# jabhinav/Semi-Supervised-Gated-LT-VAE

Measured on NVIDIA B200. Metric: training images/sec (sup+unsup ELBO step), higher is better.
Workload: dtype bf16

## Files before the change

semi-supervised-gated-lt-vae_b200/csrc/conv_tc.cu:

```cuda
#include <stdlib.h>
#include <string.h>

#include <mutex>
#include <type_traits>

#include "common.cuh"
#include "tc_common.cuh"

namespace gccvae {
using namespace tc;

__device__ __forceinline__ size_t s2d_slot(int n, int y, int x, int H, int W) {
  const int HB = (H >> 1) + 1, WB = (W >> 1) + 1;
  return (((size_t)n * HB + ((y + 1) >> 1)) * WB + ((x + 1) >> 1)) * 4 + (((y + 1) & 1) * 2 + ((x + 1) & 1));
}

struct alignas(64) TapGemmParams {
  CUtensorMap tmA, tmB;
  int num_taps, chunks, KC, swz;
  int a_scale;
  int BW, BH, BN;
  int tiles_w, tiles_h;
  int N, n_store;
  int b_tap_stride;
  short a_dw[4][16], a_dh[4][16];
  int b_row0[4];
  void* out;
  const void* mask;
  const float* bias;
  int bias_mod;
  int act;
  int out_f32;
  int OH, OW, OC, oys, oxs;
  int oy0[4], ox0[4];
  int batch;
  int stages;
  int tps;
  int n_slabs;
  int phases;
  int total_items;
  int bias_n;
  long long* timeline;
  int out_s2d, mask_s2d;
  int rows_valid;
  int pad_;
  int halo2;
  int a_box_rows;
};

#ifdef GCCVAE_TIMELINE
#define TL_ON(p) ((p).timeline != nullptr)
#define TL(item_local, slot)                                                              \
  do {                                                                                    \
    if (p.timeline != nullptr && blockIdx.x == 0 && (item_local) < 32)                    \
      p.timeline[(item_local) * 8 + (slot)] = clock64();                                  \
  } while (0)
#else
#define TL_ON(p) false
#define TL(item_local, slot) \
  do {                       \
  } while (0)
#endif

constexpr int TG_THREADS = 192;

__global__ void __launch_bounds__(TG_THREADS) tapgemm_kernel(const __grid_constant__ TapGemmParams p) {
  extern __shared__ uint8_t smem_raw[];
  const uint32_t base = (smem_u32(smem_raw) + 1023u) & ~1023u;
  uint8_t* smem = smem_raw + (base - smem_u32(smem_raw));
  const int a_bytes = p.a_box_rows * p.KC * 2, b_tile = p.N * p.KC * 2, b_bytes = (p.halo2 ? 2 : 1) * b_tile;
  const int a_stride = (a_bytes + 1023) & ~1023, b_stride = (b_bytes + 1023) & ~1023;
  const int stage_stride = p.tps * (a_stride + b_stride);
  uint8_t* sA = smem;
  uint8_t* sB = smem + p.tps * a_stride;
  uint64_t* full = reinterpret_cast<uint64_t*>(smem + p.stages * stage_stride);
  uint64_t* empty = full + p.stages;
  uint64_t* tfull = empty + p.stages;
  uint64_t* tempty = tfull + 2;
  uint32_t* tmem_slot = reinterpret_cast<uint32_t*>(tempty + 2);
  float* s_bias = reinterpret_cast<float*>((reinterpret_cast<uintptr_t>(tmem_slot + 4) + 15) & ~(uintptr_t)15);

  const int warp = threadIdx.x >> 5, lane = threadIdx.x & 31;
  pdl_launch_dependents();
  const int per_cta = (p.total_items + (int)gridDim.x - 1) / (int)gridDim.x;
  const int item_beg = blockIdx.x * per_cta;
  const int item_end = min(item_beg + per_cta, p.total_items);
  const int tiles_per_group = p.tiles_w * p.tiles_h;
  uint32_t acc_cols = 32;
  while ((int)acc_cols < p.N) acc_cols <<= 1;
  const uint32_t tmem_cols = acc_cols * 2;

  if (warp == 0 && lane == 0) {
    tma_prefetch_desc(&p.tmA);
    tma_prefetch_desc(&p.tmB);
    for (int s = 0; s < p.stages; ++s) {
      mbar_init(&full[s], 1);
      mbar_init(&empty[s], 1);
    }
    for (int s = 0; s < 2; ++s) {
      mbar_init(&tfull[s], 1);
      mbar_init(&tempty[s], 4);
    }
    fence_mbar_init();
  }
  if (warp == 2) tmem_alloc(tmem_slot, tmem_cols);
  tc_fence_before();
  __syncthreads();
  tc_fence_after();
  const uint32_t tmem_base = *tmem_slot;
  pdl_wait();
  if (TL_ON(p) && threadIdx.x == 0 && blockIdx.x < 1024) {
    unsigned long long gt;
    asm volatile("mov.u64 %0, %globaltimer;" : "=l"(gt));
    p.timeline[40 * 8 + 2 * blockIdx.x] = (long long)gt;
  }

  const int k_iters = p.num_taps * p.chunks;
  if (warp == 0) {
    if (elect_one()) {
      int stage = 0;
      uint32_t ph = 0;
      long long prod_wait = 0;
      const long long tp0 = clock64();
      const uint32_t stage_tx =
          (uint32_t)(p.tps * ((p.halo2 ? p.a_box_rows : p.rows_valid) * p.KC * 2 + b_bytes));
      for (int item = item_beg; item < item_end; ++item) {
        const int phase_id = item % p.phases, slab = (item / p.phases) % p.n_slabs, tile = item / (p.phases * p.n_slabs);
        const int grp = tile / tiles_per_group, tin = tile % tiles_per_group;
        const int w0 = (tin % p.tiles_w) * p.BW, h0 = (tin / p.tiles_w) * p.BH, n0 = grp * p.BN;
        const int aw = p.a_scale * w0, ah = p.a_scale * h0, brow = p.b_row0[phase_id] + slab * p.N;
        int t = 0, c = 0;
        for (int it = 0; it < k_iters; it += p.tps) {
          const long long tw0 = TL_ON(p) ? clock64() : 0;
          mbar_wait(&empty[stage], ph ^ 1);
          if (TL_ON(p)) prod_wait += clock64() - tw0;
          if (it == 0) TL(item - item_beg, 0);
          mbar_expect_tx(&full[stage], stage_tx);
          uint8_t* a_dst = sA + stage * stage_stride;
          uint8_t* b_dst = sB + stage * stage_stride;
          for (int j = 0; j < p.tps; ++j) {
            tma_load_4d(a_dst, &p.tmA, &full[stage], c * p.KC, aw + p.a_dw[phase_id][t], ah + p.a_dh[phase_id][t], n0);
            if (p.halo2) {
              tma_load_2d(b_dst, &p.tmB, &full[stage], t * p.b_tap_stride + c * p.KC, brow);
              tma_load_2d(b_dst + b_tile, &p.tmB, &full[stage], (2 + t) * p.b_tap_stride + c * p.KC, brow);
            } else {
              tma_load_2d(b_dst, &p.tmB, &full[stage], t * p.b_tap_stride + c * p.KC, brow);
            }
            a_dst += a_stride;
            b_dst += b_stride;
            if (++c == p.chunks) { c = 0; ++t; }
          }
          if (it + p.tps >= k_iters) TL(item - item_beg, 1);
          if (++stage == p.stages) { stage = 0; ph ^= 1; }
        }
      }
      if (TL_ON(p) && blockIdx.x == 0) {
        p.timeline[32 * 8 + 0] = prod_wait;
        p.timeline[32 * 8 + 1] = clock64() - tp0;
      }
    }
  } else if (warp == 1) {
    if (lane == 0) {
      const uint32_t idesc = instr_desc_bf16(128, p.N, 0, 0);
      const uint32_t sbo = 8u * (uint32_t)p.KC * 2u;
      const uint64_t dproto = smem_desc(0, 16, sbo, (uint32_t)p.swz);
      const uint64_t adesc0 = dproto + (uint64_t)(smem_u32(sA) >> 4), bdesc0 = dproto + (uint64_t)(smem_u32(sB) >> 4);
      const uint32_t a_step = (uint32_t)a_stride >> 4, b_step = (uint32_t)b_stride >> 4;
      const uint32_t st_step = (uint32_t)stage_stride >> 4;
      const int kk_n = p.KC / 16;
      int stage = 0;
      uint32_t ph = 0;
      long long mma_wait = 0, acc_wait = 0;
      const long long tm0 = clock64();
      auto run = [&](auto kk_c) {
      constexpr int KK = decltype(kk_c)::value;
      for (int item = item_beg; item < item_end; ++item) {
        const int li = item - item_beg, as = li & 1;
        const long long ta0 = TL_ON(p) ? clock64() : 0;
        mbar_wait(&tempty[as], ((uint32_t)(li >> 1) & 1u) ^ 1u);
        if (TL_ON(p)) acc_wait += clock64() - ta0;
        tc_fence_after();
        TL(li, 2);
        const uint32_t tacc = tmem_base + (uint32_t)as * acc_cols;
        for (int it = 0; it < k_iters; it += p.tps) {
          const long long tw0 = TL_ON(p) ? clock64() : 0;
          mbar_wait(&full[stage], ph);
          if (TL_ON(p)) mma_wait += clock64() - tw0;
          tc_fence_after();
          if (it + p.tps >= k_iters) TL(li, 3);
          uint64_t ad = adesc0 + (uint64_t)((uint32_t)stage * st_step);
          uint64_t bd = bdesc0 + (uint64_t)((uint32_t)stage * st_step);
          if (p.halo2) {
            const uint32_t a_shift = (uint32_t)(p.BW * p.KC * 2) >> 4, b_shift = (uint32_t)b_tile >> 4;
            for (int j = 0; j < p.tps; ++j) {
              for (int a = 0; a < 2; ++a)
#pragma unroll
                for (int kk = 0; kk < KK; ++kk)
                  umma_bf16(tacc, ad + (uint64_t)(a * a_shift + 2u * kk), bd + (uint64_t)(a * b_shift + 2u * kk), idesc,
                            (it > 0 || j > 0 || a > 0 || kk > 0) ? 1u : 0u);
              ad += a_step;
              bd += b_step;
            }
          } else {
          umma_bf16(tacc, ad, bd, idesc, it > 0 ? 1u : 0u);
#pragma unroll
          for (int kk = 1; kk < KK; ++kk) umma_bf16(tacc, ad + 2u * kk, bd + 2u * kk, idesc, 1u);
          for (int j = 1; j < p.tps; ++j) {
            ad += a_step;
            bd += b_step;
#pragma unroll
            for (int kk = 0; kk < KK; ++kk) umma_bf16(tacc, ad + 2u * kk, bd + 2u * kk, idesc, 1u);
          }
          }
          umma_commit(&empty[stage]);
          if (it + p.tps >= k_iters) umma_commit(&tfull[as]);
          if (++stage == p.stages) { stage = 0; ph ^= 1; }
        }
      }
      };
      if (kk_n == 4) run(std::integral_constant<int, 4>{});
      else if (kk_n == 2) run(std::integral_constant<int, 2>{});
      else run(std::integral_constant<int, 1>{});
      if (TL_ON(p) && blockIdx.x == 0) {
        p.timeline[32 * 8 + 2] = mma_wait;
        p.timeline[32 * 8 + 3] = acc_wait;
        p.timeline[32 * 8 + 4] = clock64() - tm0;
        p.timeline[32 * 8 + 5] = (long long)(item_end - item_beg) * (k_iters / p.tps);
        p.timeline[32 * 8 + 6] = p.stages;
        p.timeline[32 * 8 + 7] = gridDim.x;
      }
    }
  } else {
    const int q = warp & 3;
    const int m = q * 32 + lane;
    const int dx = m % p.BW, dy = (m / p.BW) % p.BH, dn = m / (p.BW * p.BH);
    {
      const int nb = p.bias == nullptr ? 0 : (p.bias_mod < p.bias_n ? p.bias_mod : p.bias_n);
      for (int i = threadIdx.x - 64; i < 256; i += 128) s_bias[i] = i < nb ? p.bias[i] : 0.0f;
      asm volatile("bar.sync 1, 128;" ::: "memory");
    }
    for (int item = item_beg; item < item_end; ++item) {
      const int li = item - item_beg, as = li & 1;
      const int phase_id = item % p.phases, slab = (item / p.phases) % p.n_slabs, tile = item / (p.phases * p.n_slabs);
      const int grp = tile / tiles_per_group, tin = tile % tiles_per_group;
      const int w0 = (tin % p.tiles_w) * p.BW, h0 = (tin / p.tiles_w) * p.BH, n0 = grp * p.BN;
      const int slab0 = slab * p.N;
      const int n = n0 + dn, y = h0 + dy, x = w0 + dx;
      const bool valid = n < p.batch && m < p.rows_valid;
      const int oyy = y * p.oys + p.oy0[phase_id], oxx = x * p.oxs + p.ox0[phase_id];
      const size_t opix_lin = ((size_t)n * p.OH + (size_t)oyy) * p.OW + oxx;
      const size_t opix_s2d = (p.out_s2d | p.mask_s2d) ? s2d_slot(n, oyy, oxx, p.OH, p.OW) : 0;
      const size_t opix = p.out_s2d ? opix_s2d : opix_lin;
      const size_t mpix = p.mask_s2d ? opix_s2d : opix_lin;
      const uint32_t tacc = tmem_base + (uint32_t)as * acc_cols + ((uint32_t)(q * 32) << 16);
      uint32_t mpre[4][8];
      const bool use_mask = p.mask != nullptr && valid;
      if (use_mask) {
        const __nv_bfloat16* mk = reinterpret_cast<const __nv_bfloat16*>(p.mask) + mpix * p.OC + slab0;
#pragma unroll
        for (int i = 0; i < 4; ++i)
          if (i * 16 < p.N && slab0 + i * 16 < p.n_store) ld_global_nc_256(mk + i * 16, mpre[i]);
      }
      mbar_wait(&tfull[as], (uint32_t)(li >> 1) & 1u);
      tc_fence_after();
      if (threadIdx.x == 64) TL(li, 4);
      const int bias_base = slab0 % p.bias_mod;
      const uint32_t s_bias_u32 = smem_u32(s_bias);
      for (int c0 = 0; c0 < p.N; c0 += 16) {
        const int cg = slab0 + c0;
        const uint32_t bsrc = s_bias_u32 + (uint32_t)(((bias_base + c0) & 255) * 4);
        uint32_t r[16];
        tmem_ld16(tacc + (uint32_t)c0, r);
        tmem_ld_wait();
        if (c0 + 16 >= p.N) {
          tc_fence_before();
          if (lane == 0) mbar_arrive(&tempty[as]);
          if (threadIdx.x == 64) TL(li, 5);
        }
        if (!valid || cg >= p.n_store) continue;
        float v[16];
#pragma unroll
        for (int i = 0; i < 4; ++i) {
          const float4 t = lds_f4(bsrc + 16u * i);
          v[4 * i] = __uint_as_float(r[4 * i]) + t.x;
          v[4 * i + 1] = __uint_as_float(r[4 * i + 1]) + t.y;
          v[4 * i + 2] = __uint_as_float(r[4 * i + 2]) + t.z;
          v[4 * i + 3] = __uint_as_float(r[4 * i + 3]) + t.w;
        }
        if (p.act == GCCVAE_ACT_RELU) {
#pragma unroll
          for (int i = 0; i < 16; ++i) v[i] = fmaxf(v[i], 0.0f);
        } else if (p.act == GCCVAE_ACT_SIGMOID) {
          if (p.out_f32 == 2) {
#pragma unroll
            for (int i = 0; i < 3; ++i) v[i] = __fdividef(1.0f, 1.0f + __expf(-v[i]));
          } else {
#pragma unroll
            for (int i = 0; i < 16; ++i) v[i] = __fdividef(1.0f, 1.0f + __expf(-v[i]));
          }
        }
        const size_t o = opix * p.OC + cg;
        if (use_mask) {
          uint32_t mw[8];
          if (c0 < 64) {
            switch (c0 >> 4) {
              case 0:
#pragma unroll
                for (int i = 0; i < 8; ++i) mw[i] = mpre[0][i];
                break;
              case 1:
#pragma unroll
                for (int i = 0; i < 8; ++i) mw[i] = mpre[1][i];
                break;
              case 2:
#pragma unroll
                for (int i = 0; i < 8; ++i) mw[i] = mpre[2][i];
                break;
              default:
#pragma unroll
                for (int i = 0; i < 8; ++i) mw[i] = mpre[3][i];
                break;
            }
          } else {
            ld_global_nc_256(reinterpret_cast<const __nv_bfloat16*>(p.mask) + mpix * p.OC + cg, mw);
          }
#pragma unroll
          for (int i = 0; i < 8; ++i) {
            const uint32_t lo = mw[i] & 0xffffu, hi = mw[i] >> 16;
            if (!(lo != 0 && lo < 0x8000u)) v[2 * i] = 0.0f;
            if (!(hi != 0 && hi < 0x8000u)) v[2 * i + 1] = 0.0f;
          }
        }
        if (p.out_f32 == 2) {
          if (c0 == 0) reinterpret_cast<float4*>(p.out)[opix] = make_float4(v[0], v[1], v[2], 0.0f);
        } else if (p.out_f32) {
          float* dst = reinterpret_cast<float*>(p.out) + o;
          uint32_t w0[8], w1[8];
#pragma unroll
          for (int i = 0; i < 8; ++i) { w0[i] = __float_as_uint(v[i]); w1[i] = __float_as_uint(v[8 + i]); }
          st_global_256(dst, w0);
          st_global_256(dst + 8, w1);
        } else {
          uint32_t w[8];
#pragma unroll
          for (int i = 0; i < 8; ++i) w[i] = pack_bf16x2(v[2 * i], v[2 * i + 1]);
          st_global_256(reinterpret_cast<__nv_bfloat16*>(p.out) + o, w);
        }
      }
      if (threadIdx.x == 64) TL(li, 6);
    }
    tc_fence_before();
  }
  __syncthreads();
  if (TL_ON(p) && threadIdx.x == 0 && blockIdx.x < 1024) {
    unsigned long long gt;
    asm volatile("mov.u64 %0, %globaltimer;" : "=l"(gt));
    p.timeline[40 * 8 + 2 * blockIdx.x + 1] = (long long)gt;
  }
  if (warp == 2) {
    tc_fence_after();
    tmem_dealloc(tmem_base, tmem_cols);
  }
}

struct alignas(64) SlHaloParams {
  CUtensorMap tmA, tmB;
  int C, BW, BH, tiles_h;
  int N, n_store, swz;
  void* out;
  const void* mask;
  const float* bias;
  int bias_n, act, out_f32;
  int OH, OW, OC, batch, total_tiles, stages;
  long long* timeline;
  int mask_s2d;
};
constexpr int HALO_THREADS = 320;

__global__ void __launch_bounds__(HALO_THREADS) sl_halo_kernel(const __grid_constant__ SlHaloParams p) {
  extern __shared__ uint8_t smem_raw[];
  const uint32_t base = (smem_u32(smem_raw) + 1023u) & ~1023u;
  uint8_t* smem = smem_raw + (base - smem_u32(smem_raw));
  const int rowb = p.C * 2;
  const int avb = (p.BH + 2) * p.BW * rowb;
  const int a_stage = 3 * avb;
  const int bblk = 4 * p.N * rowb;
  uint8_t* sB = smem;
  uint8_t* sA = smem + ((9 * bblk + 1023) & ~1023);
  uint64_t* full = reinterpret_cast<uint64_t*>(sA + p.stages * a_stage);
  uint64_t* empty = full + p.stages;
  uint64_t* tfull = empty + p.stages;
  uint64_t* tempty = tfull + 2;
  uint64_t* bfull = tempty + 2;
  uint32_t* tmem_slot = reinterpret_cast<uint32_t*>(bfull + 1);
  float* s_bias = reinterpret_cast<float*>((reinterpret_cast<uintptr_t>(tmem_slot + 4) + 15) & ~(uintptr_t)15);

  const int warp = threadIdx.x >> 5, lane = threadIdx.x & 31;
  pdl_launch_dependents();
  const int per_cta = (p.total_tiles + (int)gridDim.x - 1) / (int)gridDim.x;
  const int tile_beg = blockIdx.x * per_cta;
  const int tile_end = min(tile_beg + per_cta, p.total_tiles);
  uint32_t tmem_cols = 32;
  while ((int)tmem_cols < 8 * p.N) tmem_cols <<= 1;

  if (warp == 0 && lane == 0) {
    tma_prefetch_desc(&p.tmA);
    tma_prefetch_desc(&p.tmB);
    for (int s = 0; s < p.stages; ++s) {
      mbar_init(&full[s], 1);
      mbar_init(&empty[s], 1);
    }
    for (int s = 0; s < 2; ++s) {
      mbar_init(&tfull[s], 1);
      mbar_init(&tempty[s], 8);
    }
    mbar_init(bfull, 1);
    fence_mbar_init();
  }
  if (warp == 2) tmem_alloc(tmem_slot, tmem_cols);
  for (int i = threadIdx.x; i < 256; i += HALO_THREADS)
    s_bias[i] = (p.bias != nullptr && i < p.bias_n) ? p.bias[i] : 0.0f;
  tc_fence_before();
  __syncthreads();
  tc_fence_after();
  const uint32_t tmem_base = *tmem_slot;
  pdl_wait();

  if (warp == 0) {
    if (elect_one() && tile_beg < tile_end) {
      mbar_expect_tx(bfull, (uint32_t)(9 * bblk));
      for (int view = 0; view < 9; ++view)
        tma_load_2d(sB + view * bblk, &p.tmB, bfull, 0, view * 4 * p.N);
      int stage = 0;
      uint32_t ph = 0;
      for (int tile = tile_beg; tile < tile_end; ++tile) {
        const int n = tile / p.tiles_h, h0 = (tile % p.tiles_h) * p.BH;
        mbar_wait(&empty[stage], ph ^ 1);
        TL(tile - tile_beg, 0);
        mbar_expect_tx(&full[stage], (uint32_t)a_stage);
        for (int v = 0; v < 3; ++v)
          tma_load_4d(sA + stage * a_stage + v * avb, &p.tmA, &full[stage], 0, v - 1, h0 - 1, n);
// ... 1211 lines not shown
  });
  return fn;
}

static CUtensorMapSwizzle tma_swizzle_for(int inner_bytes) {
  return inner_bytes >= 128 ? CU_TENSOR_MAP_SWIZZLE_128B
         : inner_bytes >= 64 ? CU_TENSOR_MAP_SWIZZLE_64B
         : inner_bytes >= 32 ? CU_TENSOR_MAP_SWIZZLE_32B
                             : CU_TENSOR_MAP_SWIZZLE_NONE;
}
static int umma_swizzle_for(int inner_bytes) {
  return inner_bytes >= 128 ? SW_128 : inner_bytes >= 64 ? SW_64 : inner_bytes >= 32 ? SW_32 : SW_NONE;
}

static int encode_act_map(CUtensorMap* m, const void* ptr, int N, int H, int W, int C, int kc, int bw, int bh, int bn,
                          int es) {
  EncodeTiledFn enc = get_encode();
  if (!enc) {
    set_error("cuTensorMapEncodeTiled is unavailable (driver too old?)");
    return GCCVAE_ECUDA;
  }
  cuuint64_t dims[4] = {(cuuint64_t)C, (cuuint64_t)W, (cuuint64_t)H, (cuuint64_t)N};
  cuuint64_t strides[3] = {(cuuint64_t)C * 2, (cuuint64_t)W * C * 2, (cuuint64_t)H * W * C * 2};
  cuuint32_t box[4] = {(cuuint32_t)kc, (cuuint32_t)(bw * es), (cuuint32_t)(bh * es), (cuuint32_t)bn};
  cuuint32_t estr[4] = {1, (cuuint32_t)es, (cuuint32_t)es, 1};
  CUresult r = enc(m, CU_TENSOR_MAP_DATA_TYPE_BFLOAT16, 4, const_cast<void*>(ptr), dims, strides, box, estr,
                   CU_TENSOR_MAP_INTERLEAVE_NONE, tma_swizzle_for(kc * 2), CU_TENSOR_MAP_L2_PROMOTION_L2_128B,
                   CU_TENSOR_MAP_FLOAT_OOB_FILL_NONE);
  if (r != CUDA_SUCCESS) {
    set_error("cuTensorMapEncodeTiled(act %dx%dx%dx%d box %d,%d,%d,%d es %d) failed: %d", N, H, W, C, kc, bw * es,
              bh * es, bn, es, (int)r);
    return GCCVAE_ECUDA;
  }
  return GCCVAE_OK;
}

static int encode_mat_map(CUtensorMap* m, const void* ptr, long long rows, long long K, int kc, int nrows) {
  EncodeTiledFn enc = get_encode();
  if (!enc) {
    set_error("cuTensorMapEncodeTiled is unavailable (driver too old?)");
    return GCCVAE_ECUDA;
  }
  cuuint64_t dims[2] = {(cuuint64_t)K, (cuuint64_t)rows};
  cuuint64_t strides[1] = {(cuuint64_t)K * 2};
  cuuint32_t box[2] = {(cuuint32_t)kc, (cuuint32_t)nrows};
  cuuint32_t estr[2] = {1, 1};
  CUresult r = enc(m, CU_TENSOR_MAP_DATA_TYPE_BFLOAT16, 2, const_cast<void*>(ptr), dims, strides, box, estr,
                   CU_TENSOR_MAP_INTERLEAVE_NONE, tma_swizzle_for(kc * 2), CU_TENSOR_MAP_L2_PROMOTION_L2_128B,
                   CU_TENSOR_MAP_FLOAT_OOB_FILL_NONE);
  if (r != CUDA_SUCCESS) {
    set_error("cuTensorMapEncodeTiled(mat %lldx%lld box %d,%d) failed: %d", rows, K, kc, nrows, (int)r);
    return GCCVAE_ECUDA;
  }
  return GCCVAE_OK;
}

static int pick_kc(int C) {
  if (C % 64 == 0) return 64;
  if (C == 32) return 32;
  if (C == 16) return 16;
  return 0;
}

static int pick_tile(int H, int W, int* bw, int* bh, int* bn) {
  if (W >= 128 || 128 % W != 0) return -1;
  *bw = W;
  int rest = 128 / W;
  if (H >= rest) {
    if (H % rest != 0) return -1;
    *bh = rest;
    *bn = 1;
  } else {
    if (rest % H != 0) return -1;
    *bh = H;
    *bn = rest / H;
  }
  return 0;
}

constexpr int WG_PER_SM = 2, WG_SMEM_KB = 100;

template <class Params>
static cudaError_t launch_pdl(void (*kernel)(const Params), dim3 grid, int threads, size_t smem, cudaStream_t st,
                              const Params& p) {
  cudaLaunchConfig_t cfg;
  memset(&cfg, 0, sizeof(cfg));
  cfg.gridDim = grid;
  cfg.blockDim = dim3(threads, 1, 1);
  cfg.dynamicSmemBytes = smem;
  cfg.stream = st;
  cudaLaunchAttribute attr[1];
  attr[0].id = cudaLaunchAttributeProgrammaticStreamSerialization;
  attr[0].val.programmaticStreamSerializationAllowed = 1;
  cfg.attrs = attr;
  cfg.numAttrs = 1;
  return cudaLaunchKernelEx(&cfg, kernel, p);
}

static long long* g_timeline = nullptr;

static int launch_tapgemm(TapGemmParams& p, int groups, int phases, cudaStream_t st, const char* name) {
  p.timeline = g_timeline;
  if (p.rows_valid <= 0) p.rows_valid = 128;
  if (p.a_box_rows <= 0) p.a_box_rows = 128;
  const int a_stride = (p.a_box_rows * p.KC * 2 + 1023) & ~1023,
            b_stride = ((p.halo2 ? 2 : 1) * p.N * p.KC * 2 + 1023) & ~1023;
  uint32_t acc_cols = 32;
  while ((int)acc_cols < p.N) acc_cols <<= 1;
  const int k_iters = p.num_taps * p.chunks;
  int per_sm = 2;
  if (per_sm > 512 / (2 * (int)acc_cols)) per_sm = 512 / (2 * (int)acc_cols);
  if (per_sm < 1) per_sm = 1;
  const int budget = 200 * 1024 / per_sm - 4608;
  const int stage_target = 48 * 1024;
  int tps = 1;
  for (int d = 1; d <= k_iters; ++d)
    if (k_iters % d == 0 && d * (a_stride + b_stride) <= stage_target && 2 * d * (a_stride + b_stride) <= budget) tps = d;
  p.tps = tps;
  int stages = budget / (tps * (a_stride + b_stride));
  if (stages > 8) stages = 8;
  if (stages < 2) stages = 2;
  p.stages = stages;
  const size_t smem = (size_t)stages * tps * (a_stride + b_stride) + 1024 + 256 + 2048 + 64;
  static bool attr_set = false;
  if (!attr_set) {
    GCC_CUDA(cudaFuncSetAttribute(tapgemm_kernel, cudaFuncAttributeMaxDynamicSharedMemorySize, (int)(200 * 1024)));
    attr_set = true;
  }
  GCC_REQUIRE(smem <= 200 * 1024, "%s: %zu bytes of shared memory", name, smem);
  if (p.n_slabs < 1) p.n_slabs = 1;
  if (p.bias_mod < 1 || p.bias == nullptr) p.bias_mod = 1 << 30;
  if (p.bias_n < 1) p.bias_n = p.n_store;
  GCC_REQUIRE(p.bias_mod >= p.n_store || p.bias_mod % p.N == 0, "%s: bias_mod %d incompatible with N slab %d", name,
              p.bias_mod, p.N);
  GCC_REQUIRE(p.bias == nullptr || ((uintptr_t)p.bias % 16) == 0, "%s: bias must be 16-byte aligned", name);
  p.phases = phases;
  p.total_items = groups * p.tiles_w * p.tiles_h * p.n_slabs * phases;
  static int regs_per_cta = 0;
  if (regs_per_cta == 0) {
    cudaFuncAttributes fa;
    GCC_CUDA(cudaFuncGetAttributes(&fa, tapgemm_kernel));
    const int per_warp = ((fa.numRegs + 7) / 8) * 8 * 32;
    regs_per_cta = per_warp * (TG_THREADS / 32);
  }
  int occ = 65536 / regs_per_cta;
  const int occ_smem = (int)((227 * 1024) / (smem + 1024));
  if (occ > occ_smem) occ = occ_smem;
  if (occ < 1) occ = 1;
  if (per_sm > occ) per_sm = occ;
  if (getenv("GCCVAE_DEBUG_LAUNCH"))
    fprintf(stderr, "%s: N=%d KC=%d k_iters=%d tps=%d stages=%d smem=%zu per_sm=%d (occ %d) items=%d\n", name, p.N, p.KC,
            k_iters, tps, stages, smem, per_sm, occ, p.total_items);
  int ctas = p.total_items < 148 * per_sm ? p.total_items : 148 * per_sm;
  {
    const int per_cta = (p.total_items + ctas - 1) / ctas;
    ctas = (p.total_items + per_cta - 1) / per_cta;
  }
  dim3 grid(ctas, 1, 1);
  GCC_CUDA(launch_pdl(tapgemm_kernel, grid, TG_THREADS, smem, st, p));
  GCC_CHECK_LAUNCH(name);
  return GCCVAE_OK;
}

}

using namespace gccvae;

extern "C" int gccvae_ls_bf16(const gccvae_geom* g, const void* L, const void* Wp_ls, const float* bias, int act,
                              const void* mask, void* S, int out_f32, void* stream) {
  GCC_REQUIRE(g && L && Wp_ls && S, "ls_bf16: null pointer");
  const int kc = pick_kc(g->CL);
  GCC_REQUIRE(kc > 0, "ls_bf16: CL=%d unsupported (need 16, 32 or a multiple of 64)", g->CL);
  GCC_REQUIRE(g->CS % 16 == 0 && g->CS <= 256, "ls_bf16: CS=%d must be a multiple of 16, <= 256", g->CS);
  TapGemmParams p;
  memset(&p, 0, sizeof(p));
  const bool dense = (g->HS == 1 && g->WS == 1 && g->pad == 0 && g->stride == 1);
  int rc, n_slab = g->CS;
  if (dense) {
    const int Kt = g->KH * g->KW * g->CL;
    if ((rc = encode_act_map(&p.tmA, L, g->batch, 1, 1, Kt, kc, 1, 1, 128, 1))) return rc;
    p.num_taps = 1; p.chunks = Kt / kc; p.a_scale = 1; p.BW = 1; p.BH = 1; p.BN = 128; p.tiles_w = p.tiles_h = 1;
    p.b_tap_stride = 0;
    const int m_tiles = (g->batch + 127) / 128;
    n_slab = (m_tiles < 74 && g->CS % 64 == 0 && g->CS > 64) ? 64 : g->CS;
    if ((rc = encode_mat_map(&p.tmB, Wp_ls, g->CS, Kt, kc, n_slab))) return rc;
  } else {
    GCC_REQUIRE(g->KH == 4 && g->KW == 4 && g->stride == 2 && g->pad == 1, "ls_bf16: only k4/s2/p1 or dense");
    int bw, bh, bn;
    GCC_REQUIRE(pick_tile(g->HS, g->WS, &bw, &bh, &bn) == 0, "ls_bf16: cannot tile %dx%d", g->HS, g->WS);
    if ((rc = encode_act_map(&p.tmA, L, g->batch, g->HL, g->WL, g->CL, kc, bw, bh, bn, 2))) return rc;
    p.num_taps = 16; p.chunks = g->CL / kc; p.a_scale = 2; p.BW = bw; p.BH = bh; p.BN = bn;
    p.tiles_w = g->WS / bw; p.tiles_h = g->HS / bh;
    for (int t = 0; t < 16; ++t) { p.a_dh[0][t] = (short)(t / 4 - 1); p.a_dw[0][t] = (short)(t % 4 - 1); }
    p.b_tap_stride = g->CL;
    if ((rc = encode_mat_map(&p.tmB, Wp_ls, g->CS, 16LL * g->CL, kc, g->CS))) return rc;
  }
  p.KC = kc; p.swz = umma_swizzle_for(kc * 2);
  p.N = n_slab; p.n_store = g->CS; p.n_slabs = g->CS / n_slab;
  p.out = S; p.mask = mask; p.bias = bias; p.act = act & ~GCCVAE_LAYOUT_FLAGS; p.out_f32 = out_f32;
  p.out_s2d = (act & GCCVAE_OUT_S2D) ? 1 : 0; p.mask_s2d = (act & GCCVAE_MASK_S2D) ? 1 : 0;
  GCC_REQUIRE(!p.out_s2d || (out_f32 == 0 && !dense), "ls_bf16: s2d output needs a bf16 spatial output");
  p.OH = g->HS; p.OW = g->WS; p.OC = g->CS; p.oys = p.oxs = 1;
  p.batch = g->batch;
  const int groups = (g->batch + p.BN - 1) / p.BN;
  return launch_tapgemm(p, groups, 1, (cudaStream_t)stream, "ls_bf16");
}

extern "C" int gccvae_sl_bf16(const gccvae_geom* g, const void* S, const void* Wp_sl, const float* bias, int act,
                              const void* mask, void* L, int out_f32, void* stream) {
  GCC_REQUIRE(g && S && Wp_sl && L, "sl_bf16: null pointer");
  const int kc = pick_kc(g->CS);
  GCC_REQUIRE(kc > 0, "sl_bf16: CS=%d unsupported (need 16, 32 or a multiple of 64)", g->CS);
  TapGemmParams p;
  memset(&p, 0, sizeof(p));
  int rc, phases;
  const bool dense = (g->HS == 1 && g->WS == 1 && g->pad == 0 && g->stride == 1);
  if (dense) {
    const int Nt = g->KH * g->KW * g->CL;
    const int nslab = Nt <= 256 ? Nt : (Nt % 256 == 0 ? 256 : (Nt % 128 == 0 ? 128 : 0));
    GCC_REQUIRE(nslab > 0 && nslab % 16 == 0, "sl_bf16(dense): N=%d unsupported", Nt);
    phases = 1;
    if ((rc = encode_act_map(&p.tmA, S, g->batch, 1, 1, g->CS, kc, 1, 1, 128, 1))) return rc;
    p.num_taps = 1; p.chunks = g->CS / kc; p.a_scale = 1; p.BW = 1; p.BH = 1; p.BN = 128; p.tiles_w = p.tiles_h = 1;
    if ((rc = encode_mat_map(&p.tmB, Wp_sl, Nt, g->CS, kc, nslab))) return rc;
    p.N = nslab; p.n_store = Nt; p.n_slabs = Nt / nslab;
    p.OH = 1; p.OW = 1; p.OC = Nt; p.oys = p.oxs = 1;
    p.bias_mod = g->CL;
  } else {
    GCC_REQUIRE(g->KH == 4 && g->KW == 4 && g->stride == 2 && g->pad == 1, "sl_bf16: only k4/s2/p1 or dense");
    int bw, bh, bn;
    GCC_REQUIRE(pick_tile(g->HS, g->WS, &bw, &bh, &bn) == 0, "sl_bf16: cannot tile %dx%d", g->HS, g->WS);
    const int rows_pad = (g->CL + 15) / 16 * 16;
    GCC_REQUIRE(rows_pad <= 256, "sl_bf16: CL too large");
    GCC_REQUIRE(g->CL % 16 == 0 || (g->CL == 3 && out_f32 == 2 && mask == nullptr),
                "sl_bf16: CL=%d must be a multiple of 16 (or 3 with the float4 image output)", g->CL);
    phases = 4;
    if ((rc = encode_act_map(&p.tmA, S, g->batch, g->HS, g->WS, g->CS, kc, bw, bh, bn, 1))) return rc;
    p.num_taps = 4; p.chunks = g->CS / kc; p.a_scale = 1; p.BW = bw; p.BH = bh; p.BN = bn;
    p.tiles_w = g->WS / bw; p.tiles_h = g->HS / bh;
    for (int z = 0; z < 4; ++z) {
      const int ph = z >> 1, pw = z & 1;
      for (int t = 0; t < 4; ++t) { p.a_dh[z][t] = (short)(ph - (t >> 1)); p.a_dw[z][t] = (short)(pw - (t & 1)); }
// ... 579 lines not shown
```

semi-supervised-gated-lt-vae_b200/csrc/tc_common.cuh:

```cuda
#pragma once
#include <cuda.h>
#include <cuda_bf16.h>
#include <cuda_runtime.h>
#include <stdint.h>

namespace gccvae {
namespace tc {

__device__ __forceinline__ uint32_t smem_u32(const void* p) { return (uint32_t)__cvta_generic_to_shared(p); }
__device__ __forceinline__ float4 lds_f4(uint32_t smem_addr) {
  float4 v;
  asm volatile("ld.shared.v4.f32 {%0, %1, %2, %3}, [%4];" : "=f"(v.x), "=f"(v.y), "=f"(v.z), "=f"(v.w) : "r"(smem_addr));
  return v;
}

__device__ __forceinline__ bool elect_one() {
  uint32_t pred;
  asm volatile(
      "{\n\t.reg .pred p;\n\t.reg .b32 r;\n\telect.sync r|p, 0xffffffff;\n\tselp.u32 %0, 1, 0, p;\n\t}\n"
      : "=r"(pred));
  return pred != 0;
}

__device__ __forceinline__ void mbar_init(uint64_t* bar, uint32_t count) {
  asm volatile("mbarrier.init.shared::cta.b64 [%0], %1;" ::"r"(smem_u32(bar)), "r"(count));
}
__device__ __forceinline__ void fence_mbar_init() { asm volatile("fence.mbarrier_init.release.cluster;" ::: "memory"); }
__device__ __forceinline__ void mbar_expect_tx(uint64_t* bar, uint32_t bytes) {
  asm volatile("mbarrier.arrive.expect_tx.shared::cta.b64 _, [%0], %1;" ::"r"(smem_u32(bar)), "r"(bytes) : "memory");
}
__device__ __forceinline__ void mbar_arrive(uint64_t* bar) {
  asm volatile("mbarrier.arrive.shared::cta.b64 _, [%0];" ::"r"(smem_u32(bar)) : "memory");
}
__device__ __forceinline__ void mbar_wait(uint64_t* bar, uint32_t parity) {
  const uint32_t addr = smem_u32(bar);
  for (uint32_t spin = 0;; ++spin) {
    uint32_t done;
    asm volatile(
        "{\n\t.reg .pred p;\n\tmbarrier.try_wait.parity.shared::cta.b64 p, [%1], %2;\n\tselp.u32 %0, 1, 0, p;\n\t}\n"
        : "=r"(done)
        : "r"(addr), "r"(parity)
        : "memory");
    if (done) return;
    if (spin > (1u << 24)) {
      printf("gccvae: mbarrier wait timed out (block %d,%d,%d thread %d)\n", blockIdx.x, blockIdx.y, blockIdx.z,
             threadIdx.x);
      __trap();
    }
  }
}

__device__ __forceinline__ void mbar_wait_relaxed(uint64_t* bar, uint32_t parity) {
  const uint32_t addr = smem_u32(bar);
  uint32_t ns = 32;
  for (uint32_t spin = 0;; ++spin) {
    uint32_t done;
    asm volatile(
        "{\n\t.reg .pred p;\n\tmbarrier.try_wait.parity.shared::cta.b64 p, [%1], %2;\n\tselp.u32 %0, 1, 0, p;\n\t}\n"
        : "=r"(done)
        : "r"(addr), "r"(parity)
        : "memory");
    if (done) return;
    __nanosleep(ns);
    if (ns < 512) ns <<= 1;
    if (spin > (1u << 22)) {
      printf("gccvae: mbarrier wait (relaxed) timed out (block %d thread %d)\n", blockIdx.x, threadIdx.x);
      __trap();
    }
  }
}

__device__ __forceinline__ void tma_prefetch_desc(const CUtensorMap* m) {
  asm volatile("prefetch.tensormap [%0];" ::"l"(m) : "memory");
}
__device__ __forceinline__ void tma_load_2d(void* dst, const CUtensorMap* m, uint64_t* bar, int c0, int c1) {
  asm volatile(
      "cp.async.bulk.tensor.2d.shared::cluster.global.tile.mbarrier::complete_tx::bytes [%0], [%1, {%3, %4}], [%2];"
      ::"r"(smem_u32(dst)), "l"(m), "r"(smem_u32(bar)), "r"(c0), "r"(c1)
      : "memory");
}
__device__ __forceinline__ void tma_load_4d(void* dst, const CUtensorMap* m, uint64_t* bar, int c0, int c1, int c2,
                                            int c3) {
  asm volatile(
      "cp.async.bulk.tensor.4d.shared::cluster.global.tile.mbarrier::complete_tx::bytes [%0], [%1, {%3, %4, %5, %6}], "
      "[%2];" ::"r"(smem_u32(dst)),
      "l"(m), "r"(smem_u32(bar)), "r"(c0), "r"(c1), "r"(c2), "r"(c3)
      : "memory");
}

__device__ __forceinline__ void bulk_load_1d(void* dst, const void* src, uint32_t bytes, uint64_t* bar) {
  asm volatile("cp.async.bulk.shared::cluster.global.mbarrier::complete_tx::bytes [%0], [%1], %2, [%3];" ::"r"(smem_u32(dst)),
               "l"(src), "r"(bytes), "r"(smem_u32(bar))
               : "memory");
}
__device__ __forceinline__ uint4 lds_u4(uint32_t smem_addr) {
  uint4 v;
  asm volatile("ld.shared.v4.u32 {%0, %1, %2, %3}, [%4];" : "=r"(v.x), "=r"(v.y), "=r"(v.z), "=r"(v.w) : "r"(smem_addr));
  return v;
}

__device__ __forceinline__ void tmem_alloc(uint32_t* dst_smem, uint32_t ncols) {
  asm volatile("tcgen05.alloc.cta_group::1.sync.aligned.shared::cta.b32 [%0], %1;" ::"r"(smem_u32(dst_smem)),
               "r"(ncols)
               : "memory");
  asm volatile("tcgen05.relinquish_alloc_permit.cta_group::1.sync.aligned;" ::: "memory");
}
__device__ __forceinline__ void tmem_dealloc(uint32_t addr, uint32_t ncols) {
  asm volatile("tcgen05.dealloc.cta_group::1.sync.aligned.b32 %0, %1;" ::"r"(addr), "r"(ncols) : "memory");
}
__device__ __forceinline__ void tc_fence_before() { asm volatile("tcgen05.fence::before_thread_sync;" ::: "memory"); }
__device__ __forceinline__ void tc_fence_after() { asm volatile("tcgen05.fence::after_thread_sync;" ::: "memory"); }

__device__ __forceinline__ void umma_bf16(uint32_t tmem_d, uint64_t adesc, uint64_t bdesc, uint32_t idesc,
                                          uint32_t accumulate) {
  asm volatile(
      "{\n\t.reg .pred p;\n\tsetp.ne.b32 p, %4, 0;\n\t"
      "tcgen05.mma.cta_group::1.kind::f16 [%0], %1, %2, %3, p;\n\t}\n" ::"r"(tmem_d),
      "l"(adesc), "l"(bdesc), "r"(idesc), "r"(accumulate)
      : "memory");
}
__device__ __forceinline__ void umma_commit(uint64_t* bar) {
  asm volatile("tcgen05.commit.cta_group::1.mbarrier::arrive::one.shared::cluster.b64 [%0];" ::"r"(smem_u32(bar))
               : "memory");
}
__device__ __forceinline__ void tmem_ld16(uint32_t taddr, uint32_t (&r)[16]) {
  asm volatile(
      "tcgen05.ld.sync.aligned.32x32b.x16.b32 {%0,%1,%2,%3,%4,%5,%6,%7,%8,%9,%10,%11,%12,%13,%14,%15}, [%16];"
      : "=r"(r[0]), "=r"(r[1]), "=r"(r[2]), "=r"(r[3]), "=r"(r[4]), "=r"(r[5]), "=r"(r[6]), "=r"(r[7]), "=r"(r[8]),
        "=r"(r[9]), "=r"(r[10]), "=r"(r[11]), "=r"(r[12]), "=r"(r[13]), "=r"(r[14]), "=r"(r[15])
      : "r"(taddr)
      : "memory");
}
__device__ __forceinline__ void tmem_ld_wait() { asm volatile("tcgen05.wait::ld.sync.aligned;" ::: "memory"); }

enum Swizzle : uint32_t { SW_NONE = 0, SW_128 = 2, SW_64 = 4, SW_32 = 6 };

__device__ __forceinline__ uint64_t smem_desc(uint32_t saddr, uint32_t lbo_bytes, uint32_t sbo_bytes, uint32_t layout) {
  uint64_t d = 0;
  d |= (uint64_t)((saddr >> 4) & 0x3FFF);
  d |= (uint64_t)((lbo_bytes >> 4) & 0x3FFF) << 16;
  d |= (uint64_t)((sbo_bytes >> 4) & 0x3FFF) << 32;
  d |= (uint64_t)1 << 46;
  d |= (uint64_t)(layout & 7) << 61;
  return d;
}
__host__ __device__ __forceinline__ uint32_t instr_desc_bf16(int M, int N, int a_mn_major, int b_mn_major) {
  uint32_t d = 0;
  d |= 1u << 4;
  d |= 1u << 7;
  d |= 1u << 10;
  d |= (uint32_t)(a_mn_major & 1) << 15;
  d |= (uint32_t)(b_mn_major & 1) << 16;
  d |= (uint32_t)(N >> 3) << 17;
  d |= (uint32_t)(M >> 4) << 24;
// ... 25 lines not shown
```

Before: 1.726 million.

## Add cluster split-K with DSMEM reduction for dense low-tile tap GEMMs

Adds a templated split-K path to the tcgen05 tap-GEMM kernel for dense (1x1 tap, 1x1 spatial block) GEMMs with long K and few output tiles. The K loop is divided across 2 or 4 CTAs in a thread-block cluster, and partial accumulators are exchanged through distributed shared memory guarded by cluster mbarriers. Each CTA then reduces and stores its own column slice. This aims to fill more SMs when there are too few output items to occupy the GPU, at the cost of extra DSMEM traffic, cluster synchronisation and reduction shared memory. It also sets launch bounds to 2 blocks per SM and changes the shared-memory budget for small grids.

New measurement: 1.778 million (median of 6 runs). +3.0%, better.

```diff
diff --git a/semi-supervised-gated-lt-vae_b200/csrc/conv_tc.cu b/semi-supervised-gated-lt-vae_b200/csrc/conv_tc.cu
--- a/semi-supervised-gated-lt-vae_b200/csrc/conv_tc.cu
+++ b/semi-supervised-gated-lt-vae_b200/csrc/conv_tc.cu
@@ -46,6 +46,7 @@
   int pad_;
   int halo2;
   int a_box_rows;
+  int split;
 };
 
 #ifdef GCCVAE_TIMELINE
@@ -64,7 +65,8 @@
 
 constexpr int TG_THREADS = 192;
 
-__global__ void __launch_bounds__(TG_THREADS) tapgemm_kernel(const __grid_constant__ TapGemmParams p) {
+template <bool SPLIT>
+__global__ void __launch_bounds__(TG_THREADS, 2) tapgemm_kernel(const __grid_constant__ TapGemmParams p) {
   extern __shared__ uint8_t smem_raw[];
   const uint32_t base = (smem_u32(smem_raw) + 1023u) & ~1023u;
   uint8_t* smem = smem_raw + (base - smem_u32(smem_raw));
@@ -77,13 +79,19 @@
   uint64_t* empty = full + p.stages;
   uint64_t* tfull = empty + p.stages;
   uint64_t* tempty = tfull + 2;
-  uint32_t* tmem_slot = reinterpret_cast<uint32_t*>(tempty + 2);
+  uint64_t* rfull = tempty + 2;
+  uint64_t* rfree = rfull + 1;
+  uint32_t* tmem_slot = reinterpret_cast<uint32_t*>(rfree + 1);
   float* s_bias = reinterpret_cast<float*>((reinterpret_cast<uintptr_t>(tmem_slot + 4) + 15) & ~(uintptr_t)15);
+  float* s_red = s_bias + 256;
 
   const int warp = threadIdx.x >> 5, lane = threadIdx.x & 31;
   pdl_launch_dependents();
-  const int per_cta = (p.total_items + (int)gridDim.x - 1) / (int)gridDim.x;
-  const int item_beg = blockIdx.x * per_cta;
+  const int split = SPLIT ? p.split : 1;
+  const uint32_t crank = split > 1 ? cluster_ctarank() : 0u;
+  const int units = (int)gridDim.x / split;
+  const int per_cta = (p.total_items + units - 1) / units;
+  const int item_beg = ((int)blockIdx.x / split) * per_cta;
   const int item_end = min(item_beg + per_cta, p.total_items);
   const int tiles_per_group = p.tiles_w * p.tiles_h;
   uint32_t acc_cols = 32;
@@ -101,11 +109,16 @@
       mbar_init(&tfull[s], 1);
       mbar_init(&tempty[s], 4);
     }
+    if (split > 1) {
+      mbar_init(rfull, (split - 1) * 128);
+      mbar_init(rfree, (split - 1) * 128);
+    }
     fence_mbar_init();
   }
   if (warp == 2) tmem_alloc(tmem_slot, tmem_cols);
   tc_fence_before();
   __syncthreads();
+  if (split > 1) cluster_sync();
   tc_fence_after();
   const uint32_t tmem_base = *tmem_slot;
   pdl_wait();
@@ -115,7 +128,7 @@
     p.timeline[40 * 8 + 2 * blockIdx.x] = (long long)gt;
   }
 
-  const int k_iters = p.num_taps * p.chunks;
+  const int k_iters = p.num_taps * p.chunks / split, k_beg = (int)crank * k_iters;
   if (warp == 0) {
     if (elect_one()) {
       int stage = 0;
@@ -129,7 +142,7 @@
         const int grp = tile / tiles_per_group, tin = tile % tiles_per_group;
         const int w0 = (tin % p.tiles_w) * p.BW, h0 = (tin / p.tiles_w) * p.BH, n0 = grp * p.BN;
         const int aw = p.a_scale * w0, ah = p.a_scale * h0, brow = p.b_row0[phase_id] + slab * p.N;
-        int t = 0, c = 0;
+        int t = k_beg / p.chunks, c = k_beg % p.chunks;
         for (int it = 0; it < k_iters; it += p.tps) {
           const long long tw0 = TL_ON(p) ? clock64() : 0;
           mbar_wait(&empty[stage], ph ^ 1);
@@ -239,6 +252,8 @@
       for (int i = threadIdx.x - 64; i < 256; i += 128) s_bias[i] = i < nb ? p.bias[i] : 0.0f;
       asm volatile("bar.sync 1, 128;" ::: "memory");
     }
+    const int ncol = p.N / split, col_beg = (int)crank * ncol, col_end = col_beg + ncol;
+    const uint32_t red_slot = (uint32_t)ncol * 512u, s_red_m = smem_u32(s_red) + (uint32_t)m * 16u;
     for (int item = item_beg; item < item_end; ++item) {
       const int li = item - item_beg, as = li & 1;
       const int phase_id = item % p.phases, slab = (item / p.phases) % p.n_slabs, tile = item / (p.phases * p.n_slabs);
@@ -256,26 +271,61 @@
       uint32_t mpre[4][8];
       const bool use_mask = p.mask != nullptr && valid;
       if (use_mask) {
-        const __nv_bfloat16* mk = reinterpret_cast<const __nv_bfloat16*>(p.mask) + mpix * p.OC + slab0;
+        const __nv_bfloat16* mk = reinterpret_cast<const __nv_bfloat16*>(p.mask) + mpix * p.OC + slab0 + col_beg;
 #pragma unroll
         for (int i = 0; i < 4; ++i)
-          if (i * 16 < p.N && slab0 + i * 16 < p.n_store) ld_global_nc_256(mk + i * 16, mpre[i]);
+          if (i * 16 < ncol && slab0 + col_beg + i * 16 < p.n_store) ld_global_nc_256(mk + i * 16, mpre[i]);
       }
       mbar_wait(&tfull[as], (uint32_t)(li >> 1) & 1u);
       tc_fence_after();
       if (threadIdx.x == 64) TL(li, 4);
+      if (split > 1) {
+        if (li > 0) mbar_wait_cluster(rfree, (uint32_t)(li - 1) & 1u);
+        for (int k = 1; k < split; ++k) {
+          const uint32_t dst = (crank + (uint32_t)k) % (uint32_t)split;
+          const uint32_t slot = crank - (crank > dst ? 1u : 0u);
+          const uint32_t rdst = mapa_shared(s_red_m + slot * red_slot, dst);
+          for (int c = 0; c < ncol; c += 16) {
+            uint32_t r[16];
+            tmem_ld16(tacc + dst * (uint32_t)ncol + (uint32_t)c, r);
+            tmem_ld_wait();
+#pragma unroll
+            for (int i = 0; i < 4; ++i)
+              st_cluster_v4(rdst + (uint32_t)((c / 4 + i) * 128) * 16u, r[4 * i], r[4 * i + 1], r[4 * i + 2], r[4 * i + 3]);
+          }
+        }
+        for (int k = 1; k < split; ++k) mbar_arrive_cluster(mapa_shared(smem_u32(rfull), (crank + (uint32_t)k) % (uint32_t)split));
+        mbar_wait_cluster(rfull, (uint32_t)li & 1u);
+      }
       const int bias_base = slab0 % p.bias_mod;
       const uint32_t s_bias_u32 = smem_u32(s_bias);
-      for (int c0 = 0; c0 < p.N; c0 += 16) {
+      for (int c0 = col_beg; c0 < col_end; c0 += 16) {
         const int cg = slab0 + c0;
         const uint32_t bsrc = s_bias_u32 + (uint32_t)(((bias_base + c0) & 255) * 4);
         uint32_t r[16];
         tmem_ld16(tacc + (uint32_t)c0, r);
         tmem_ld_wait();
-        if (c0 + 16 >= p.N) {
+        if (c0 + 16 >= col_end) {
           tc_fence_before();
           if (lane == 0) mbar_arrive(&tempty[as]);
           if (threadIdx.x == 64) TL(li, 5);
+        }
+        if (split > 1) {
+          const uint32_t src0 = s_red_m + (uint32_t)(((c0 - col_beg) / 4) * 128) * 16u;
+#pragma unroll
+          for (int i = 0; i < 4; ++i) {
+            float4 a = make_float4(__uint_as_float(r[4 * i]), __uint_as_float(r[4 * i + 1]), __uint_as_float(r[4 * i + 2]),
+                                   __uint_as_float(r[4 * i + 3]));
+            const float4 own = a;
+            for (int k = 0; k < split; ++k) {
+              const float4 b = k == (int)crank ? own
+                                               : lds_f4(src0 + (uint32_t)(k - (k > (int)crank ? 1 : 0)) * red_slot +
+                                                        (uint32_t)(i * 128) * 16u);
+              if (k == 0) { a = b; } else { a.x += b.x; a.y += b.y; a.z += b.z; a.w += b.w; }
+            }
+            r[4 * i] = __float_as_uint(a.x); r[4 * i + 1] = __float_as_uint(a.y);
+            r[4 * i + 2] = __float_as_uint(a.z); r[4 * i + 3] = __float_as_uint(a.w);
+          }
         }
         if (!valid || cg >= p.n_store) continue;
         float v[16];
@@ -302,8 +352,8 @@
         const size_t o = opix * p.OC + cg;
         if (use_mask) {
           uint32_t mw[8];
-          if (c0 < 64) {
-            switch (c0 >> 4) {
+          if (c0 - col_beg < 64) {
+            switch ((c0 - col_beg) >> 4) {
               case 0:
 #pragma unroll
                 for (int i = 0; i < 8; ++i) mw[i] = mpre[0][i];
@@ -347,6 +397,7 @@
           st_global_256(reinterpret_cast<__nv_bfloat16*>(p.out) + o, w);
         }
       }
+      for (int k = 1; k < split; ++k) mbar_arrive_cluster(mapa_shared(smem_u32(rfree), (crank + (uint32_t)k) % (uint32_t)split));
       if (threadIdx.x == 64) TL(li, 6);
     }
     tc_fence_before();
@@ -357,6 +408,7 @@
     asm volatile("mov.u64 %0, %globaltimer;" : "=l"(gt));
     p.timeline[40 * 8 + 2 * blockIdx.x + 1] = (long long)gt;
   }
+  if (split > 1) cluster_sync();
   if (warp == 2) {
     tc_fence_after();
     tmem_dealloc(tmem_base, tmem_cols);
@@ -1734,36 +1786,55 @@
 
 template <class Params>
 static cudaError_t launch_pdl(void (*kernel)(const Params), dim3 grid, int threads, size_t smem, cudaStream_t st,
-                              const Params& p) {
+                              const Params& p, int cluster = 1) {
   cudaLaunchConfig_t cfg;
   memset(&cfg, 0, sizeof(cfg));
   cfg.gridDim = grid;
   cfg.blockDim = dim3(threads, 1, 1);
   cfg.dynamicSmemBytes = smem;
   cfg.stream = st;
-  cudaLaunchAttribute attr[1];
+  cudaLaunchAttribute attr[2];
   attr[0].id = cudaLaunchAttributeProgrammaticStreamSerialization;
   attr[0].val.programmaticStreamSerializationAllowed = 1;
+  attr[1].id = cudaLaunchAttributeClusterDimension;
+  attr[1].val.clusterDim.x = (unsigned)cluster;
+  attr[1].val.clusterDim.y = 1;
+  attr[1].val.clusterDim.z = 1;
   cfg.attrs = attr;
-  cfg.numAttrs = 1;
+  cfg.numAttrs = cluster > 1 ? 2 : 1;
   return cudaLaunchKernelEx(&cfg, kernel, p);
 }
 
 static long long* g_timeline = nullptr;
+
+static int tapgemm_split(const TapGemmParams& p, int phases) {
+  const int k_blocks = p.num_taps * p.chunks;
+  const bool dense = p.num_taps == 1 && p.BW == 1 && p.BH == 1;
+  if (phases != 1 || !dense || k_blocks < 16 || p.n_store % 64 != 0) return 1;
+  return k_blocks >= 32 ? 4 : 2;
+}
 
 static int launch_tapgemm(TapGemmParams& p, int groups, int phases, cudaStream_t st, const char* name) {
   p.timeline = g_timeline;
   if (p.rows_valid <= 0) p.rows_valid = 128;
   if (p.a_box_rows <= 0) p.a_box_rows = 128;
+  if (p.n_slabs < 1) p.n_slabs = 1;
+  p.phases = phases;
+  p.total_items = groups * p.tiles_w * p.tiles_h * p.n_slabs * phases;
+  const int split = tapgemm_split(p, phases);
+  p.split = split;
+  const int k_iters = p.num_taps * p.chunks / split;
+  GCC_REQUIRE(k_iters * split == p.num_taps * p.chunks && p.N % (16 * split) == 0, "%s: split %d of K=%d, N=%d", name,
+              split, p.num_taps * p.chunks, p.N);
+  const int red_bytes = (split - 1) * 128 * (p.N / split) * 4;
   const int a_stride = (p.a_box_rows * p.KC * 2 + 1023) & ~1023,
             b_stride = ((p.halo2 ? 2 : 1) * p.N * p.KC * 2 + 1023) & ~1023;
   uint32_t acc_cols = 32;
   while ((int)acc_cols < p.N) acc_cols <<= 1;
-  const int k_iters = p.num_taps * p.chunks;
   int per_sm = 2;
   if (per_sm > 512 / (2 * (int)acc_cols)) per_sm = 512 / (2 * (int)acc_cols);
   if (per_sm < 1) per_sm = 1;
-  const int budget = 200 * 1024 / per_sm - 4608;
+  const int budget = 200 * 1024 / (p.total_items * split <= 148 ? 1 : per_sm) - 4608 - red_bytes;
   const int stage_target = 48 * 1024;
   int tps = 1;
   for (int d = 1; d <= k_iters; ++d)
@@ -1773,43 +1844,70 @@
   if (stages > 8) stages = 8;
   if (stages < 2) stages = 2;
   p.stages = stages;
-  const size_t smem = (size_t)stages * tps * (a_stride + b_stride) + 1024 + 256 + 2048 + 64;
+  const size_t smem = (size_t)stages * tps * (a_stride + b_stride) + 1024 + 256 + 2048 + 64 + red_bytes;
+  void (*kernel)(const TapGemmParams) = split > 1 ? tapgemm_kernel<true> : tapgemm_kernel<false>;
   static bool attr_set = false;
   if (!attr_set) {
-    GCC_CUDA(cudaFuncSetAttribute(tapgemm_kernel, cudaFuncAttributeMaxDynamicSharedMemorySize, (int)(200 * 1024)));
+    GCC_CUDA(cudaFuncSetAttribute(tapgemm_kernel<false>, cudaFuncAttributeMaxDynamicSharedMemorySize, (int)(200 * 1024)));
+    GCC_CUDA(cudaFuncSetAttribute(tapgemm_kernel<true>, cudaFuncAttributeMaxDynamicSharedMemorySize, (int)(200 * 1024)));
     attr_set = true;
   }
   GCC_REQUIRE(smem <= 200 * 1024, "%s: %zu bytes of shared memory", name, smem);
-  if (p.n_slabs < 1) p.n_slabs = 1;
   if (p.bias_mod < 1 || p.bias == nullptr) p.bias_mod = 1 << 30;
   if (p.bias_n < 1) p.bias_n = p.n_store;
   GCC_REQUIRE(p.bias_mod >= p.n_store || p.bias_mod % p.N == 0, "%s: bias_mod %d incompatible with N slab %d", name,
               p.bias_mod, p.N);
   GCC_REQUIRE(p.bias == nullptr || ((uintptr_t)p.bias % 16) == 0, "%s: bias must be 16-byte aligned", name);
-  p.phases = phases;
-  p.total_items = groups * p.tiles_w * p.tiles_h * p.n_slabs * phases;
-  static int regs_per_cta = 0;
-  if (regs_per_cta == 0) {
+  static int regs_per_cta[2] = {0, 0};
+  int& regs = regs_per_cta[split > 1];
+  if (regs == 0) {
     cudaFuncAttributes fa;
-    GCC_CUDA(cudaFuncGetAttributes(&fa, tapgemm_kernel));
+    GCC_CUDA(cudaFuncGetAttributes(&fa, kernel));
     const int per_warp = ((fa.numRegs + 7) / 8) * 8 * 32;
-    regs_per_cta = per_warp * (TG_THREADS / 32);
-  }
-  int occ = 65536 / regs_per_cta;
+    regs = per_warp * (TG_THREADS / 32);
+  }
+  int occ = 65536 / regs;
   const int occ_smem = (int)((227 * 1024) / (smem + 1024));
   if (occ > occ_smem) occ = occ_smem;
   if (occ < 1) occ = 1;
   if (per_sm > occ) per_sm = occ;
+  int max_units = 148 * per_sm / split;
+  if (split > 1) {
+    static std::mutex mu;
+    static int cached[3][2] = {{0, 0}, {0, 0}, {0, 0}};
+    std::lock_guard<std::mutex> lock(mu);
+    int* c = cached[split / 2];
+    if (c[0] != (int)smem) {
+      cudaLaunchConfig_t cfg;
+      memset(&cfg, 0, sizeof(cfg));
+      cfg.gridDim = dim3(split * max_units, 1, 1);
+      cfg.blockDim = dim3(TG_THREADS, 1, 1);
+      cfg.dynamicSmemBytes = smem;
+      cudaLaunchAttribute attr;
+      attr.id = cudaLaunchAttributeClusterDimension;
+      attr.val.clusterDim.x = (unsigned)split;
+      attr.val.clusterDim.y = 1;
+      attr.val.clusterDim.z = 1;
+      cfg.attrs = &attr;
+      cfg.numAttrs = 1;
+      int n = 0;
+      GCC_CUDA(cudaOccupancyMaxActiveClusters(&n, kernel, &cfg));
+      c[0] = (int)smem;
+      c[1] = n;
+    }
+    if (c[1] > 0 && max_units > c[1]) max_units = c[1];
+  }
+  if (max_units < 1) max_units = 1;
+  int units = p.total_items < max_units ? p.total_items : max_units;
+  {
+    const int per_unit = (p.total_items + units - 1) / units;
+    units = (p.total_items + per_unit - 1) / per_unit;
+  }
   if (getenv("GCCVAE_DEBUG_LAUNCH"))
-    fprintf(stderr, "%s: N=%d KC=%d k_iters=%d tps=%d stages=%d smem=%zu per_sm=%d (occ %d) items=%d\n", name, p.N, p.KC,
-            k_iters, tps, stages, smem, per_sm, occ, p.total_items);
-  int ctas = p.total_items < 148 * per_sm ? p.total_items : 148 * per_sm;
-  {
-    const int per_cta = (p.total_items + ctas - 1) / ctas;
-    ctas = (p.total_items + per_cta - 1) / per_cta;
-  }
-  dim3 grid(ctas, 1, 1);
-  GCC_CUDA(launch_pdl(tapgemm_kernel, grid, TG_THREADS, smem, st, p));
+    fprintf(stderr, "%s: N=%d KC=%d k_iters=%d tps=%d stages=%d smem=%zu per_sm=%d (occ %d) items=%d split=%d clusters=%d\n",
+            name, p.N, p.KC, k_iters, tps, stages, smem, per_sm, occ, p.total_items, split, split > 1 ? units : 0);
+  dim3 grid(units * split, 1, 1);
+  GCC_CUDA(launch_pdl(kernel, grid, TG_THREADS, smem, st, p, split));
   GCC_CHECK_LAUNCH(name);
   return GCCVAE_OK;
 }
diff --git a/semi-supervised-gated-lt-vae_b200/csrc/tc_common.cuh b/semi-supervised-gated-lt-vae_b200/csrc/tc_common.cuh
--- a/semi-supervised-gated-lt-vae_b200/csrc/tc_common.cuh
+++ b/semi-supervised-gated-lt-vae_b200/csrc/tc_common.cuh
@@ -70,6 +70,44 @@
   }
 }
 
+__device__ __forceinline__ uint32_t cluster_ctarank() {
+  uint32_t r;
+  asm volatile("mov.u32 %0, %%cluster_ctarank;" : "=r"(r));
+  return r;
+}
+__device__ __forceinline__ uint32_t mapa_shared(uint32_t smem_addr, uint32_t rank) {
+  uint32_t r;
+  asm volatile("mapa.shared::cluster.u32 %0, %1, %2;" : "=r"(r) : "r"(smem_addr), "r"(rank));
+  return r;
+}
+__device__ __forceinline__ void st_cluster_v4(uint32_t cluster_addr, uint32_t a, uint32_t b, uint32_t c, uint32_t d) {
+  asm volatile("st.shared::cluster.v4.b32 [%0], {%1, %2, %3, %4};" ::"r"(cluster_addr), "r"(a), "r"(b), "r"(c), "r"(d)
+               : "memory");
+}
+__device__ __forceinline__ void mbar_arrive_cluster(uint32_t cluster_addr) {
+  asm volatile("mbarrier.arrive.release.cluster.shared::cluster.b64 _, [%0];" ::"r"(cluster_addr) : "memory");
+}
+__device__ __forceinline__ void mbar_wait_cluster(uint64_t* bar, uint32_t parity) {
+  const uint32_t addr = smem_u32(bar);
+  for (uint32_t spin = 0;; ++spin) {
+    uint32_t done;
+    asm volatile(
+        "{\n\t.reg .pred p;\n\tmbarrier.try_wait.parity.acquire.cluster.shared::cta.b64 p, [%1], %2;\n\t"
+        "selp.u32 %0, 1, 0, p;\n\t}\n"
+        : "=r"(done)
+        : "r"(addr), "r"(parity)
+        : "memory");
+    if (done) return;
+    if (spin > (1u << 24)) {
+      printf("gccvae: cluster mbarrier wait timed out (block %d thread %d)\n", blockIdx.x, threadIdx.x);
+      __trap();
+    }
+  }
+}
+__device__ __forceinline__ void cluster_sync() {
+  asm volatile("barrier.cluster.arrive.release;\n\tbarrier.cluster.wait.acquire;" ::: "memory");
+}
+
 __device__ __forceinline__ void tma_prefetch_desc(const CUtensorMap* m) {
   asm volatile("prefetch.tensormap [%0];" ::"l"(m) : "memory");
 }
```
